# Renmusxd/IsingMonteCarlo

Measured on AMD Instinct MI355X. Metric: spin-op updates/sec (whole node), 32×32 TFIM, 1024 replicas at 1/2/4/8 GPUs, higher is better.
Workload: dtype u32 op words, f64 acceptance arithmetic

## Files before the change

isingmontecarlo_amd/csrc/sse_fast.hip.h:

```cpp
#pragma once

namespace sse {

#define SSE_FAST_MAX_VARS 4096u
#define LDS8(a) (reinterpret_cast<uint8_t *>(lds_raw)[(a)])
#define SSE_FAST_CLASS_J 0u
#define SSE_FAST_CLASS_G 1u
#define SSE_FAST_CLASS_H 2u

__device__ __forceinline__ uint32_t sel64(uint64_t mask, uint32_t a, uint32_t b) {
    uint32_t r;
    asm("v_cndmask_b32 %0, %1, %2, %3" : "=v"(r) : "v"(b), "v"(a), "s"(mask));
    return r;
}

__device__ __forceinline__ uint32_t bfi32(uint32_t mask, uint32_t a, uint32_t b) {
    uint32_t r;
    asm("v_bfi_b32 %0, %1, %2, %3" : "=v"(r) : "v"(mask), "v"(a), "v"(b));
    return r;
}

struct FastLds {
    uint32_t o_nb;
    uint32_t o_tab;
    uint32_t o_spin;
    uint32_t o_dummy;
    uint32_t end;
};
template <int W>
__host__ __device__ __forceinline__ FastLds fast_carve(const Lds<W> &L, const DevBatch &B) {
    FastLds F;
    uint32_t base = (L.o_edges + 3u) & ~3u;
    F.o_nb = base; base += 16;
    F.o_tab = base; base += B.Nb;
    F.o_spin = base; base += B.N;
    F.o_dummy = base; base += 64;
    F.end = base;
    return F;
}

__device__ __forceinline__ uint32_t fast_entry(const DevBatch &B, uint32_t b, uint32_t ce) {
    if (b < B.E) {
        const uint32_t a = ce & SSE_CE_VAR_MASK, c = (ce >> 15) & SSE_CE_VAR_MASK, pref = (ce >> 30) & 1u;
        return a | (c << 12) | ((pref ? 0x9u : 0x6u) << 24) | (3u << 28) | (SSE_FAST_CLASS_J << 30);
    }
    const uint32_t s1 = b - B.E;
    if (s1 < B.N) return s1 | (s1 << 12) | (0xFu << 24) | (1u << 28) | (SSE_FAST_CLASS_G << 30);
    const uint32_t v = s1 - B.N;
    return v | (v << 12) | ((B.hpos ? 0x8u : 0x1u) << 24) | (1u << 28) | (SSE_FAST_CLASS_H << 30);
}

template <int K>
__device__ __forceinline__ void diagonal_fast(const DevBatch &B, const Lds<4> &L, const FastLds &F, uint32_t r, const Rng &rng, double beta,
                                              uint32_t M, int &n_io, int &ntrans_io, uint32_t &gr, uint32_t fbmask) {
    constexpr int W = 4, NT = W * 64;
    constexpr uint32_t TS = (uint32_t)(NT * K);
    static_assert(K == 2 || K == 4, "rows p and p + 64 share one Philox call");
    const int tid = threadIdx.x, lane = tid & 63, wave = __builtin_amdgcn_readfirstlane(tid >> 6);
    uint32_t *ops = B.ops + (size_t)r * B.stride;
    const uint8_t *flipb = (fbmask ? B.flipb : reinterpret_cast<const uint8_t *>(B.ops)) + (size_t)r * B.stride;
    auto ld_word = [&](uint32_t idx) -> uint32_t {
        return row_ld(ops, idx) ^ ((uint32_t)*reinterpret_cast<const uint8_t *>(reinterpret_cast<const char *>(flipb) + (size_t)idx) & fbmask);
    };
    const uint32_t N = B.N, Nb = B.Nb, E = B.E;
    for (uint32_t i = tid; i < N; i += NT) LDSW(F.o_spin, i) = ((LDSW(L.o_state, i >> 5) >> (i & 31)) & 1u) * 0x01010101u;
    __syncthreads();

    const uint32_t ntiles = (M + TS - 1) / TS;
    int n_start = n_io, ntrans = 0;
    const uint32_t m_later = (uint32_t)((0x0101010100ull << (8 * wave)) & 0xFFFFFFFFull);
    const uint32_t m_earlier = 0x01010101u & ((1u << (8 * wave)) - 1u);
    const uint32_t spin_my = 4u * F.o_spin + (uint32_t)wave;
    const uint32_t markhi = (127u - (uint32_t)lane) << 1;

    const uint32_t dummy_w = F.o_dummy + (uint32_t)lane;
    auto evmask32 = [](uint32_t wd) -> uint32_t { return 0u - ((wd ^ (wd >> 2)) & 1u); };
    auto propagate = [&](const uint32_t (&wd)[K], uint32_t mask) {
        if (mask == 0u) return;
#pragma unroll
        for (int j = 0; j < K; ++j) {
            const uint32_t v = F.o_spin + (wd[j] >> 4) - 1u - E;
            atomicXor(&lds_raw[bfi32(evmask32(wd[j]), v, dummy_w)], mask);
        }
    };

    uint32_t wnext[K];
#pragma unroll
    for (int j = 0; j < K; ++j) wnext[j] = ld_word((uint32_t)(wave * 64 * K + j * 64 + lane));
    propagate(wnext, m_later);
    __syncthreads();
    const uint32_t lane2 = 2u * (uint32_t)lane;
    const uint32_t vM = vgpr_copy_u32(M), vM1 = vgpr_copy_u32(M + 1u), vzero = vgpr_copy_u32(0u);

    for (uint32_t tile = 0; tile < ntiles; ++tile) {
#if SSE_ROTATE_PRIO
        if ((tile & (SSE_ROTATE_PRIO - 1u)) == 0u) sse_set_prio((tile / SSE_ROTATE_PRIO) + blockIdx.x);
#endif
        uint32_t word[K];
#pragma unroll
        for (int j = 0; j < K; ++j) word[j] = wnext[j];
        const uint32_t pbase = tile * TS + (uint32_t)(wave * 64 * K + lane);
        {
            const uint32_t pn = (tile + 1 < ntiles ? pbase + TS : pbase);
#pragma unroll
            for (int j = 0; j < K; ++j) wnext[j] = ld_word(pn + (uint32_t)(j * 64));
        }
        const bool partial = tile * TS + TS > M;

        double un[K], nb[K];
        uint32_t cbv[K], neww[K], ent[K], bnd[K], rr1[K];
        uint64_t insm[K], remm[K], acc[K];
        {
            uint4 rnd = make_uint4(0, 0, 0, 0);
#pragma unroll
            for (int j = 0; j < K; ++j) {
                const uint32_t wd = word[j];
                if ((j & 1) == 0) rnd = rng.draw(SSE_TAG_DIAG, pbase + (uint32_t)(j * 64));
                const uint32_t r0 = (j & 1) ? rnd.z : rnd.x;
                rr1[j] = (j & 1) ? rnd.w : rnd.y;
                const uint64_t occm = sse_ballot(wd != 0u);
                bnd[j] = sel64(occm, (wd >> 4) - 1u, __umulhi(r0, Nb));
                ent[j] = LDSW(F.o_tab, bnd[j]);
            }
        }
        uint32_t sub0[K];
#pragma unroll
        for (int j = 0; j < K; ++j) {
            const uint32_t e = ent[j], inb = word[j] & 1u;
            const uint32_t va = e & 0xFFFu, vc = (e >> 12) & 0xFFFu;
            const uint32_t adr_a = spin_my + 4u * va, adr_c = spin_my + 4u * vc;
            const uint32_t mark = markhi | inb;
            const uint32_t ev32 = evmask32(word[j]);
            const uint32_t adr_w = bfi32(ev32, adr_a, 4u * dummy_w);
            LDS8(adr_w) = (uint8_t)mark;
            SSE_WAVE_FENCE();
            const uint32_t ea = LDS8(adr_a), ec = LDS8(adr_c);
            uint32_t sa, sc;
            const uint64_t dup = sse_ballot(((ea ^ mark) & ev32) != 0u);
            if (!dup) {
                sa = (ea ^ ((ea + lane2) >> 8)) & 1u;
                sc = (ec ^ ((ec + lane2) >> 8)) & 1u;
                SSE_WAVE_FENCE();
                LDS8(adr_w) = (uint8_t)(inb ^ 1u);
            } else {
                sa = ea & 1u; sc = ec & 1u;
                bool seen_a = false, seen_c = false;
                uint64_t m = sse_ballot(ev32 != 0u);
                while (m) {
                    const int Ls = __ffsll((long long)m) - 1;
                    m &= m - 1;
                    const bool later = lane > Ls;
                    const uint32_t vL = __builtin_amdgcn_readlane(va, Ls), inL = __builtin_amdgcn_readlane(inb, Ls);
                    if (va == vL) { sa = later ? (inL ^ 1u) : (seen_a ? sa : inL); seen_a = true; }
                    if (vc == vL) { sc = later ? (inL ^ 1u) : (seen_c ? sc : inL); seen_c = true; }
                    if (lane == Ls) LDS8(adr_a) = (uint8_t)(inL ^ 1u);
                }
                SSE_WAVE_FENCE();
            }
            sub0[j] = sa | (sc << 1);
        }
#pragma unroll
        for (int j = 0; j < K; ++j) {
            const uint32_t e = ent[j], wd = word[j];
            const uint32_t okbit = (e >> (24u + sub0[j])) & 1u;
            const uint32_t sub = sub0[j] & (e >> 28) & 3u;
            const double2 nbp = *reinterpret_cast<const double2 *>(&lds_raw[F.o_nb + 4u * (e >> 30)]);
            const double u = (double)rr1[j];
            insm[j] = sse_ballot(okbit > wd);
            if (partial) insm[j] &= sse_ballot(pbase + (uint32_t)(j * 64) < M);
            remm[j] = sse_ballot((wd & ~evmask32(wd)) != 0u);
            un[j] = u * nbp.y;
            nb[j] = nbp.x;
            cbv[j] = sel64(insm[j], vM, vM1);
            neww[j] = sel64(insm[j], ((bnd[j] + 1u) << 4) | sub | (sub << 2), vzero);
            acc[j] = 0ull;
        }

        int npref[K];
#pragma unroll
        for (int j = 0; j < K; ++j) npref[j] = n_start;
        int tot_all = 0, base = 0;
        bool first = true;
        for (;;) {
            int wtot = 0;
            bool changed = first;
#pragma unroll
            for (int j = 0; j < K; ++j) {
                const double t = (double)(int)(cbv[j] - (uint32_t)npref[j]);
                const uint64_t lt_ins = sse_ballot((double)rr1[j] * t < nb[j]);
                const uint64_t lt_rem = sse_ballot(un[j] < t);
                const uint64_t a = (lt_ins & insm[j]) | (lt_rem & remm[j]);
                changed |= a != acc[j];
                acc[j] = a;
                wtot += popc64(a & insm[j]) - popc64(a & remm[j]);
            }
            const int buf = gr & 1;
            if (lane == 0) { LDSI(L.o_tot, buf * W + wave) = wtot; LDSW(L.o_chg, buf * W + wave) = changed ? 1u : 0u; }
            __syncthreads();
            if (first) {
                propagate(word, m_earlier);
                if (tile + 1 < ntiles) propagate(wnext, m_later);
            }
            base = 0; tot_all = 0; uint32_t anychg = 0;
#pragma unroll
            for (int w2 = 0; w2 < W; ++w2) {
                const int t = __builtin_amdgcn_readfirstlane(LDSI(L.o_tot, buf * W + w2));
                if (w2 < wave) base += t;
                tot_all += t;
                anychg |= (uint32_t)__builtin_amdgcn_readfirstlane((int)LDSW(L.o_chg, buf * W + w2)) & 1u;
            }
            gr++;
            if (!first && !anychg) break;
            first = false;
            int run = n_start + base;
#pragma unroll
            for (int j = 0; j < K; ++j) {
                const uint64_t im = acc[j] & insm[j], rm = acc[j] & remm[j];
                const int ci = (int)__builtin_amdgcn_mbcnt_hi((uint32_t)(im >> 32), __builtin_amdgcn_mbcnt_lo((uint32_t)im, (uint32_t)run));
                const int cr = (int)__builtin_amdgcn_mbcnt_hi((uint32_t)(rm >> 32), __builtin_amdgcn_mbcnt_lo((uint32_t)rm, 0u));
                npref[j] = ci - cr;
                run += popc64(im) - popc64(rm);
            }
        }
        int dn = 0, dtr = 0;
#pragma unroll
        for (int j = 0; j < K; ++j) {
            const uint32_t fw = sel64(acc[j], neww[j], word[j]);
            row_st(ops, pbase + (uint32_t)(j * 64), fw);
            const uint64_t im = acc[j] & insm[j], rm = acc[j] & remm[j];
            const uint64_t trm = sse_ballot((ent[j] >> 30) == SSE_FAST_CLASS_G);
            dn += popc64(im) - popc64(rm);
            dtr += popc64(im & trm) - popc64(rm & trm);
        }
        ntrans += dtr;
        if (lane == 0 && (dtr | dn)) {
            const uint32_t ch = (tile * TS + (uint32_t)(wave * 64 * K)) / B.CH;
            if (dn) atomicAdd(&LDSW(L.o_chn, ch), (uint32_t)dn);
            if (dtr) atomicAdd(&LDSW(L.o_chtr, ch), (uint32_t)dtr);
        }
        n_start += tot_all;
    }
    __syncthreads();
    if (lane == 0) LDSI(L.o_tot, wave) = ntrans;
    __syncthreads();
    int dt = 0;
#pragma unroll
    for (int w2 = 0; w2 < W; ++w2) dt += LDSI(L.o_tot, w2);
    __syncthreads();
    ntrans_io += dt;
    n_io = n_start;
}

template <int K, int PHASE>
__global__ __launch_bounds__(256, 4) void sweep_fast_kernel(DevBatch B, SweepArgs A) {
    constexpr int W = 4, NT = W * 64;
    Lds<W> L;
    L.carve(B.N, B.nwords, B.lds_ufcap, B.E, B.has_long);
    const FastLds F = fast_carve<W>(L, B);
    const int tid = threadIdx.x;
    const uint32_t r = blockIdx.x;
#ifdef SSE_WG_TIMELINE
    if (tid == 0 && (B.dbg_flags & 32u)) { B.dbg[(size_t)r * 16 + 0] = __builtin_amdgcn_s_memrealtime(); B.dbg[(size_t)r * 16 + 2] = __builtin_amdgcn_s_getreg((4 << 0) | (0 << 6) | (31 << 11)); B.dbg[(size_t)r * 16 + 3] = __builtin_amdgcn_s_getreg((20 << 0) | (0 << 6) | (31 << 11)); }
#endif
    const double beta = A.beta ? A.beta[r] : 0.0;
    for (uint32_t i = tid; i < B.nwords; i += NT) LDSW(L.o_state, i) = B.state[(size_t)r * B.nwords + i];
    for (uint32_t i = tid; i < B.Nb; i += NT) LDSW(F.o_tab, i) = fast_entry(B, i, i < B.E ? B.edges_compact[i] : 0u);
    for (uint32_t i = tid; i < 2 * SSE_MAX_CHUNKS; i += NT) LDSW(L.o_chn, i) = B.chunks[(size_t)r * 2 * SSE_MAX_CHUNKS + i];
    if (tid < 4) {
        const double beta_nb = beta * (double)B.Nb;
        const double w = tid == 0 ? B.wJ : (tid == 1 ? B.gamma : (tid == 2 ? B.wh : 0.0));
        const double num = beta_nb * w;
        *reinterpret_cast<double *>(&lds_raw[F.o_nb + 4u * (uint32_t)tid]) = num * 4294967296.0;
        *reinterpret_cast<double *>(&lds_raw[F.o_nb + 4u * (uint32_t)tid + 2u]) = num * (1.0 / 4294967296.0);
    }
    __syncthreads();
    int n = (int)B.n[r], ntrans = (int)B.ntrans[r];
    uint32_t M = B.cutoff[r], err = B.err[r], gr = 0, last_out = 0;
    uint64_t epoch = B.epoch[r];
    uint64_t a4 = 0, a5 = 0;
    const uint32_t fbmask = (A.defer_flips && B.flipb && (A.domask & SSE_DO_DIAG) && !err && B.pend[r]) ? 0xFFu : 0u;
    for (uint64_t step = 0; step < A.nsteps; ++step) {
        if (err) break;
        if (A.domask & SSE_DO_DIAG) {
            const Rng rng = make_rng(B, r, epoch);
            diagonal_fast<K>(B, L, F, r, rng, beta, M, n, ntrans, gr, step == 0 ? fbmask : 0u);
            epoch++;
            a5 += M;
            if (A.domask & SSE_DO_GROW) {
                const uint32_t want = (uint32_t)n + (uint32_t)n / 2u;
                if (want > M) { if (want > B.cap) { err = 1u; break; } M = want; }
            }
        }
        if (A.domask & SSE_DO_LOOP) {
            __syncthreads();
            for (uint32_t i = tid; i < B.E; i += NT) LDSW(L.o_edges, i) = B.edges_compact[i];
            __syncthreads();
            const Rng rng = make_rng(B, r, epoch);
            last_out = loop_pass<W, true>(B, L, r, rng, M, n, gr, err);
            epoch++;
            a4 += last_out;
            if (err) break;
        }
    }
    __syncthreads();
    for (uint32_t i = tid; i < B.nwords; i += NT) B.state[(size_t)r * B.nwords + i] = LDSW(L.o_state, i);
    for (uint32_t i = tid; i < 2 * SSE_MAX_CHUNKS; i += NT) B.chunks[(size_t)r * 2 * SSE_MAX_CHUNKS + i] = LDSW(L.o_chn, i);
    if (tid == 0) {
        B.n[r] = (uint32_t)n; B.ntrans[r] = (uint32_t)ntrans; B.cutoff[r] = M; B.err[r] = err; B.epoch[r] = epoch;
        if (fbmask && A.nsteps) B.pend[r] = 0u;
        if (A.out_u32) A.out_u32[r] = last_out;
        uint64_t *acc = B.acc + (size_t)B.acc_row[r] * 8;
        acc[4] += a4; acc[5] += a5;
#ifdef SSE_WG_TIMELINE
        if (B.dbg_flags & 32u) B.dbg[(size_t)r * 16 + 1] = __builtin_amdgcn_s_memrealtime();
#endif
    }
}

}
```

isingmontecarlo_amd/csrc/sweep_fast.hip:

```cpp
#include "sse_device.hip.h"
namespace sse {
template <int K, int PHASE>
static hipError_t launch_fast_one(const LaunchCfg &c, const DevBatch &B, const SweepArgs &A) {
    hipError_t e = hipFuncSetAttribute(reinterpret_cast<const void *>(&sweep_fast_kernel<K, PHASE>), hipFuncAttributeMaxDynamicSharedMemorySize, (int)c.lds_bytes);
    if (e != hipSuccess) return e;
    hipLaunchKernelGGL((sweep_fast_kernel<K, PHASE>), dim3(B.R), dim3(256), c.lds_bytes, c.stream, B, A);
    return hipGetLastError();
}
hipError_t launch_sweep_fast(const LaunchCfg &c, const DevBatch &B, const SweepArgs &A) {
    if (c.W != 4 || c.mode != SSE_MODE_LDS_EDGES) return hipErrorInvalidValue;
    if (c.K == 4) return c.phase ? launch_fast_one<4, 1>(c, B, A) : launch_fast_one<4, 0>(c, B, A);
    if (c.K == 2) return launch_fast_one<2, 0>(c, B, A);
    return hipErrorInvalidValue;
}
}
```

Baseline: 162.5 billion.

## Replace f64 acceptance tests with exact integer thresholds in diagonal update

Adds an integer acceptance path. The insert test becomes a 64-bit multiply-add sign check against a precomputed constant, and the remove test compares an int against a threshold converted once per tile. This takes the f64 multiplies and compares out of the iterative prefix-sum fixed-point loop. It also packs the per-wave total and changed flag into one LDS word read as a single uint4, caches the decoded spin addresses, and tracks the chunk index incrementally instead of dividing every tile. The f64 path is kept for replicas whose capacity exceeds 2^21. The integer path must match the f64 decisions exactly, so rounding edge cases are a correctness risk.

```diff
diff --git a/isingmontecarlo_amd/csrc/sse_accept.h b/isingmontecarlo_amd/csrc/sse_accept.h
--- /dev/null
+++ b/isingmontecarlo_amd/csrc/sse_accept.h
@@ -0,0 +1,39 @@
+#pragma once
+#include <stdint.h>
+
+#if defined(__HIPCC__) || defined(__CUDACC__)
+#define SSE_ACCEPT_FN __host__ __device__ inline
+#else
+#define SSE_ACCEPT_FN inline
+#endif
+
+#define SSE_ACCEPT_MAX_DEN (1u << 21)
+#define SSE_ACCEPT_NEVER_INSERT 0x8000000000000000ull
+#define SSE_ACCEPT_NEVER_REMOVE 0x7FFFFFFF
+
+SSE_ACCEPT_FN uint64_t sse_accept_insert_const(double num) {
+    const double s = num * 4294967296.0;
+    if (!(s > 0.0)) return SSE_ACCEPT_NEVER_INSERT;
+    if (s >= 9223372036854775808.0) return 1ull;
+    uint64_t nbi = (uint64_t)s;
+    if ((double)nbi < s) nbi += 1ull;
+    return SSE_ACCEPT_NEVER_INSERT - nbi;
+}
+
+SSE_ACCEPT_FN bool sse_accept_insert(uint32_t rr1, uint32_t den, uint64_t c) {
+    return (int32_t)(((uint64_t)rr1 * (uint64_t)den + c) >> 32) >= 0;
+}
+
+SSE_ACCEPT_FN int32_t sse_accept_remove_threshold(uint32_t rr1, double num_lo) {
+    const double un = (double)rr1 * num_lo;
+#if defined(__HIP_DEVICE_COMPILE__)
+    int32_t r;
+    asm("v_cvt_i32_f64 %0, %1" : "=v"(r) : "v"(un));
+    return r;
+#else
+    if (!(un < 2147483647.0)) return SSE_ACCEPT_NEVER_REMOVE;
+    return un > 0.0 ? (int32_t)un : 0;
+#endif
+}
+
+SSE_ACCEPT_FN bool sse_accept_remove(int32_t den, int32_t thr) { return den > thr; }
diff --git a/isingmontecarlo_amd/csrc/sse_fast.hip.h b/isingmontecarlo_amd/csrc/sse_fast.hip.h
--- a/isingmontecarlo_amd/csrc/sse_fast.hip.h
+++ b/isingmontecarlo_amd/csrc/sse_fast.hip.h
@@ -1,4 +1,5 @@
 #pragma once
+#include "sse_accept.h"
 
 namespace sse {
 
@@ -22,6 +23,7 @@
 
 struct FastLds {
     uint32_t o_nb;
+    uint32_t o_xch;
     uint32_t o_tab;
     uint32_t o_spin;
     uint32_t o_dummy;
@@ -30,8 +32,10 @@
 template <int W>
 __host__ __device__ __forceinline__ FastLds fast_carve(const Lds<W> &L, const DevBatch &B) {
     FastLds F;
+    static_assert(4 * W >= 3 + 8, "o_xch: eight words behind an alignment gap of up to three, inside o_tot + o_chg");
     uint32_t base = (L.o_edges + 3u) & ~3u;
     F.o_nb = base; base += 16;
+    F.o_xch = (L.o_tot + 3u) & ~3u;
     F.o_tab = base; base += B.Nb;
     F.o_spin = base; base += B.N;
     F.o_dummy = base; base += 64;
@@ -50,7 +54,7 @@
     return v | (v << 12) | ((B.hpos ? 0x8u : 0x1u) << 24) | (1u << 28) | (SSE_FAST_CLASS_H << 30);
 }
 
-template <int K>
+template <int K, bool F64>
 __device__ __forceinline__ void diagonal_fast(const DevBatch &B, const Lds<4> &L, const FastLds &F, uint32_t r, const Rng &rng, double beta,
                                               uint32_t M, int &n_io, int &ntrans_io, uint32_t &gr, uint32_t fbmask) {
     constexpr int W = 4, NT = W * 64;
@@ -73,32 +77,33 @@
     const uint32_t spin_my = 4u * F.o_spin + (uint32_t)wave;
     const uint32_t markhi = (127u - (uint32_t)lane) << 1;
 
-    const uint32_t dummy_w = F.o_dummy + (uint32_t)lane;
+    const uint32_t dummy_b = 4u * (F.o_dummy + (uint32_t)lane);
     auto evmask32 = [](uint32_t wd) -> uint32_t { return 0u - ((wd ^ (wd >> 2)) & 1u); };
-    auto propagate = [&](const uint32_t (&wd)[K], uint32_t mask) {
+    const uint32_t spin_b = 4u * (F.o_spin - 1u - E);
+    auto decode = [&](uint32_t wd) -> uint32_t { return bfi32(evmask32(wd), spin_b + 4u * (wd >> 4), dummy_b); };
+    auto propagate = [&](const uint32_t (&vb)[K], uint32_t mask) {
         if (mask == 0u) return;
 #pragma unroll
-        for (int j = 0; j < K; ++j) {
-            const uint32_t v = F.o_spin + (wd[j] >> 4) - 1u - E;
-            atomicXor(&lds_raw[bfi32(evmask32(wd[j]), v, dummy_w)], mask);
-        }
+        for (int j = 0; j < K; ++j) atomicXor(reinterpret_cast<uint32_t *>(reinterpret_cast<char *>(lds_raw) + vb[j]), mask);
     };
 
-    uint32_t wnext[K];
-#pragma unroll
-    for (int j = 0; j < K; ++j) wnext[j] = ld_word((uint32_t)(wave * 64 * K + j * 64 + lane));
-    propagate(wnext, m_later);
+    uint32_t wnext[K], vnext[K];
+#pragma unroll
+    for (int j = 0; j < K; ++j) { wnext[j] = ld_word((uint32_t)(wave * 64 * K + j * 64 + lane)); vnext[j] = decode(wnext[j]); }
+    propagate(vnext, m_later);
     __syncthreads();
     const uint32_t lane2 = 2u * (uint32_t)lane;
     const uint32_t vM = vgpr_copy_u32(M), vM1 = vgpr_copy_u32(M + 1u), vzero = vgpr_copy_u32(0u);
+    const uint32_t vnever_hi = vgpr_copy_u32((uint32_t)(SSE_ACCEPT_NEVER_INSERT >> 32)), vnever_thr = vgpr_copy_u32((uint32_t)SSE_ACCEPT_NEVER_REMOVE);
+    uint32_t ch = (uint32_t)(wave * 64 * K) / B.CH, chpos = (uint32_t)(wave * 64 * K) % B.CH;
 
     for (uint32_t tile = 0; tile < ntiles; ++tile) {
 #if SSE_ROTATE_PRIO
         if ((tile & (SSE_ROTATE_PRIO - 1u)) == 0u) sse_set_prio((tile / SSE_ROTATE_PRIO) + blockIdx.x);
 #endif
-        uint32_t word[K];
-#pragma unroll
-        for (int j = 0; j < K; ++j) word[j] = wnext[j];
+        uint32_t word[K], vcur[K];
+#pragma unroll
+        for (int j = 0; j < K; ++j) { word[j] = wnext[j]; vcur[j] = vnext[j]; }
         const uint32_t pbase = tile * TS + (uint32_t)(wave * 64 * K + lane);
         {
             const uint32_t pn = (tile + 1 < ntiles ? pbase + TS : pbase);
@@ -107,9 +112,13 @@
         }
         const bool partial = tile * TS + TS > M;
 
+        uint32_t cbv[K], neww[K], ent[K], bnd[K], rr1[K];
+        uint64_t acci[K], accr[K];
+        uint32_t chi[K];
+        uint32_t clo[K];
+        int32_t thr[K];
         double un[K], nb[K];
-        uint32_t cbv[K], neww[K], ent[K], bnd[K], rr1[K];
-        uint64_t insm[K], remm[K], acc[K];
+        uint64_t insm[K], remm[K];
         {
             uint4 rnd = make_uint4(0, 0, 0, 0);
 #pragma unroll
@@ -130,13 +139,13 @@
             const uint32_t va = e & 0xFFFu, vc = (e >> 12) & 0xFFFu;
             const uint32_t adr_a = spin_my + 4u * va, adr_c = spin_my + 4u * vc;
             const uint32_t mark = markhi | inb;
-            const uint32_t ev32 = evmask32(word[j]);
-            const uint32_t adr_w = bfi32(ev32, adr_a, 4u * dummy_w);
+            const uint32_t adr_w = vcur[j] + (uint32_t)wave;
+            const uint64_t evm = sse_ballot(vcur[j] != dummy_b);
             LDS8(adr_w) = (uint8_t)mark;
             SSE_WAVE_FENCE();
             const uint32_t ea = LDS8(adr_a), ec = LDS8(adr_c);
             uint32_t sa, sc;
-            const uint64_t dup = sse_ballot(((ea ^ mark) & ev32) != 0u);
+            const uint64_t dup = sse_ballot(ea != mark) & evm;
             if (!dup) {
                 sa = (ea ^ ((ea + lane2) >> 8)) & 1u;
                 sc = (ec ^ ((ec + lane2) >> 8)) & 1u;
@@ -145,7 +154,7 @@
             } else {
                 sa = ea & 1u; sc = ec & 1u;
                 bool seen_a = false, seen_c = false;
-                uint64_t m = sse_ballot(ev32 != 0u);
+                uint64_t m = evm;
                 while (m) {
                     const int Ls = __ffsll((long long)m) - 1;
                     m &= m - 1;
@@ -164,81 +173,100 @@
             const uint32_t e = ent[j], wd = word[j];
             const uint32_t okbit = (e >> (24u + sub0[j])) & 1u;
             const uint32_t sub = sub0[j] & (e >> 28) & 3u;
-            const double2 nbp = *reinterpret_cast<const double2 *>(&lds_raw[F.o_nb + 4u * (e >> 30)]);
-            const double u = (double)rr1[j];
-            insm[j] = sse_ballot(okbit > wd);
-            if (partial) insm[j] &= sse_ballot(pbase + (uint32_t)(j * 64) < M);
-            remm[j] = sse_ballot((wd & ~evmask32(wd)) != 0u);
-            un[j] = u * nbp.y;
-            nb[j] = nbp.x;
-            cbv[j] = sel64(insm[j], vM, vM1);
-            neww[j] = sel64(insm[j], ((bnd[j] + 1u) << 4) | sub | (sub << 2), vzero);
-            acc[j] = 0ull;
+            const uint4 cls = *reinterpret_cast<const uint4 *>(&lds_raw[F.o_nb + 4u * (e >> 30)]);
+            const double num_lo = __hiloint2double((int)cls.w, (int)cls.z);
+            uint64_t im = sse_ballot(okbit > wd);
+            if (partial) im &= sse_ballot(pbase + (uint32_t)(j * 64) < M);
+            const uint64_t rm = sse_ballot(wd != 0u) & ~sse_ballot(vcur[j] != dummy_b);
+            if constexpr (F64) {
+                un[j] = (double)rr1[j] * num_lo;
+                nb[j] = __hiloint2double((int)cls.y, (int)cls.x);
+                insm[j] = im; remm[j] = rm;
+            } else {
+                clo[j] = cls.x;
+                chi[j] = sel64(im, cls.y, vnever_hi);
+                thr[j] = (int32_t)sel64(rm, (uint32_t)sse_accept_remove_threshold(rr1[j], num_lo), vnever_thr);
+            }
+            cbv[j] = sel64(im, vM, vM1);
+            neww[j] = sel64(im, ((bnd[j] + 1u) << 4) | sub | (sub << 2), vzero);
+            acci[j] = 0ull; accr[j] = 0ull;
         }
 
         int npref[K];
 #pragma unroll
         for (int j = 0; j < K; ++j) npref[j] = n_start;
-        int tot_all = 0, base = 0;
+        int tot_all = 0, base = 0, wtot = 0;
         bool first = true;
         for (;;) {
-            int wtot = 0;
-            bool changed = first;
+            wtot = 0;
+            uint64_t diff = 0ull;
 #pragma unroll
             for (int j = 0; j < K; ++j) {
-                const double t = (double)(int)(cbv[j] - (uint32_t)npref[j]);
-                const uint64_t lt_ins = sse_ballot((double)rr1[j] * t < nb[j]);
-                const uint64_t lt_rem = sse_ballot(un[j] < t);
-                const uint64_t a = (lt_ins & insm[j]) | (lt_rem & remm[j]);
-                changed |= a != acc[j];
-                acc[j] = a;
-                wtot += popc64(a & insm[j]) - popc64(a & remm[j]);
-            }
-            const int buf = gr & 1;
-            if (lane == 0) { LDSI(L.o_tot, buf * W + wave) = wtot; LDSW(L.o_chg, buf * W + wave) = changed ? 1u : 0u; }
+                const int t = (int)(cbv[j] - (uint32_t)npref[j]);
+                uint64_t ai, ar;
+                if constexpr (F64) {
+                    const double td = (double)t;
+                    ai = sse_ballot((double)rr1[j] * td < nb[j]) & insm[j];
+                    ar = sse_ballot(un[j] < td) & remm[j];
+                } else {
+                    ai = sse_ballot(sse_accept_insert(rr1[j], (uint32_t)t, ((uint64_t)chi[j] << 32) | clo[j]));
+                    ar = sse_ballot(sse_accept_remove(t, thr[j]));
+                }
+                diff |= (ai ^ acci[j]) | (ar ^ accr[j]);
+                acci[j] = ai; accr[j] = ar;
+                wtot += popc64(ai) - popc64(ar);
+            }
+            const bool changed = first | (diff != 0ull);
+            const uint32_t xch = F.o_xch + 4u * (gr & 1u);
+            if (lane == 0) LDSW(xch, wave) = ((uint32_t)wtot << 1) | (changed ? 1u : 0u);
             __syncthreads();
             if (first) {
-                propagate(word, m_earlier);
-                if (tile + 1 < ntiles) propagate(wnext, m_later);
-            }
-            base = 0; tot_all = 0; uint32_t anychg = 0;
+                propagate(vcur, m_earlier);
+#pragma unroll
+                for (int j = 0; j < K; ++j) vnext[j] = decode(wnext[j]);
+                if (tile + 1 < ntiles) propagate(vnext, m_later);
+            }
+            const uint4 xw = *reinterpret_cast<const uint4 *>(&lds_raw[xch]);
+            const int x4[W] = {__builtin_amdgcn_readfirstlane((int)xw.x), __builtin_amdgcn_readfirstlane((int)xw.y),
+                               __builtin_amdgcn_readfirstlane((int)xw.z), __builtin_amdgcn_readfirstlane((int)xw.w)};
+            base = 0; tot_all = 0;
 #pragma unroll
             for (int w2 = 0; w2 < W; ++w2) {
-                const int t = __builtin_amdgcn_readfirstlane(LDSI(L.o_tot, buf * W + w2));
+                const int t = x4[w2] >> 1;
                 if (w2 < wave) base += t;
                 tot_all += t;
-                anychg |= (uint32_t)__builtin_amdgcn_readfirstlane((int)LDSW(L.o_chg, buf * W + w2)) & 1u;
-            }
+            }
+            const uint32_t anychg = (uint32_t)(x4[0] | x4[1] | x4[2] | x4[3]) & 1u;
             gr++;
             if (!first && !anychg) break;
             first = false;
             int run = n_start + base;
 #pragma unroll
             for (int j = 0; j < K; ++j) {
-                const uint64_t im = acc[j] & insm[j], rm = acc[j] & remm[j];
+                const uint64_t im = acci[j], rm = accr[j];
                 const int ci = (int)__builtin_amdgcn_mbcnt_hi((uint32_t)(im >> 32), __builtin_amdgcn_mbcnt_lo((uint32_t)im, (uint32_t)run));
                 const int cr = (int)__builtin_amdgcn_mbcnt_hi((uint32_t)(rm >> 32), __builtin_amdgcn_mbcnt_lo((uint32_t)rm, 0u));
                 npref[j] = ci - cr;
                 run += popc64(im) - popc64(rm);
             }
         }
-        int dn = 0, dtr = 0;
+        const int dn = wtot;
+        int dtr = 0;
 #pragma unroll
         for (int j = 0; j < K; ++j) {
-            const uint32_t fw = sel64(acc[j], neww[j], word[j]);
+            const uint32_t fw = sel64(acci[j] | accr[j], neww[j], word[j]);
             row_st(ops, pbase + (uint32_t)(j * 64), fw);
-            const uint64_t im = acc[j] & insm[j], rm = acc[j] & remm[j];
             const uint64_t trm = sse_ballot((ent[j] >> 30) == SSE_FAST_CLASS_G);
-            dn += popc64(im) - popc64(rm);
-            dtr += popc64(im & trm) - popc64(rm & trm);
+            dtr += popc64(acci[j] & trm) - popc64(accr[j] & trm);
         }
         ntrans += dtr;
         if (lane == 0 && (dtr | dn)) {
-            const uint32_t ch = (tile * TS + (uint32_t)(wave * 64 * K)) / B.CH;
             if (dn) atomicAdd(&LDSW(L.o_chn, ch), (uint32_t)dn);
             if (dtr) atomicAdd(&LDSW(L.o_chtr, ch), (uint32_t)dtr);
         }
         n_start += tot_all;
+        chpos += TS;
+        while (chpos >= B.CH) { chpos -= B.CH; ch++; }
     }
     __syncthreads();
     if (lane == 0) LDSI(L.o_tot, wave) = ntrans;
@@ -251,7 +279,7 @@
     n_io = n_start;
 }
 
-template <int K, int PHASE>
+template <int K, int PHASE, bool F64>
 __global__ __launch_bounds__(256, 4) void sweep_fast_kernel(DevBatch B, SweepArgs A) {
     constexpr int W = 4, NT = W * 64;
     Lds<W> L;
@@ -270,7 +298,8 @@
         const double beta_nb = beta * (double)B.Nb;
         const double w = tid == 0 ? B.wJ : (tid == 1 ? B.gamma : (tid == 2 ? B.wh : 0.0));
         const double num = beta_nb * w;
-        *reinterpret_cast<double *>(&lds_raw[F.o_nb + 4u * (uint32_t)tid]) = num * 4294967296.0;
+        if constexpr (F64) *reinterpret_cast<double *>(&lds_raw[F.o_nb + 4u * (uint32_t)tid]) = num * 4294967296.0;
+        else *reinterpret_cast<uint64_t *>(&lds_raw[F.o_nb + 4u * (uint32_t)tid]) = sse_accept_insert_const(num);
         *reinterpret_cast<double *>(&lds_raw[F.o_nb + 4u * (uint32_t)tid + 2u]) = num * (1.0 / 4294967296.0);
     }
     __syncthreads();
@@ -283,7 +312,7 @@
         if (err) break;
         if (A.domask & SSE_DO_DIAG) {
             const Rng rng = make_rng(B, r, epoch);
-            diagonal_fast<K>(B, L, F, r, rng, beta, M, n, ntrans, gr, step == 0 ? fbmask : 0u);
+            diagonal_fast<K, F64>(B, L, F, r, rng, beta, M, n, ntrans, gr, step == 0 ? fbmask : 0u);
             epoch++;
             a5 += M;
             if (A.domask & SSE_DO_GROW) {
diff --git a/isingmontecarlo_amd/csrc/sweep_fast.hip b/isingmontecarlo_amd/csrc/sweep_fast.hip
--- a/isingmontecarlo_amd/csrc/sweep_fast.hip
+++ b/isingmontecarlo_amd/csrc/sweep_fast.hip
@@ -1,16 +1,20 @@
 #include "sse_device.hip.h"
 namespace sse {
-template <int K, int PHASE>
+template <int K, int PHASE, bool F64>
 static hipError_t launch_fast_one(const LaunchCfg &c, const DevBatch &B, const SweepArgs &A) {
-    hipError_t e = hipFuncSetAttribute(reinterpret_cast<const void *>(&sweep_fast_kernel<K, PHASE>), hipFuncAttributeMaxDynamicSharedMemorySize, (int)c.lds_bytes);
+    hipError_t e = hipFuncSetAttribute(reinterpret_cast<const void *>(&sweep_fast_kernel<K, PHASE, F64>), hipFuncAttributeMaxDynamicSharedMemorySize, (int)c.lds_bytes);
     if (e != hipSuccess) return e;
-    hipLaunchKernelGGL((sweep_fast_kernel<K, PHASE>), dim3(B.R), dim3(256), c.lds_bytes, c.stream, B, A);
+    hipLaunchKernelGGL((sweep_fast_kernel<K, PHASE, F64>), dim3(B.R), dim3(256), c.lds_bytes, c.stream, B, A);
     return hipGetLastError();
 }
 hipError_t launch_sweep_fast(const LaunchCfg &c, const DevBatch &B, const SweepArgs &A) {
     if (c.W != 4 || c.mode != SSE_MODE_LDS_EDGES) return hipErrorInvalidValue;
-    if (c.K == 4) return c.phase ? launch_fast_one<4, 1>(c, B, A) : launch_fast_one<4, 0>(c, B, A);
-    if (c.K == 2) return launch_fast_one<2, 0>(c, B, A);
+    const bool f64 = B.cap > SSE_ACCEPT_MAX_DEN;
+    if (c.K == 4) {
+        if (f64) return c.phase ? launch_fast_one<4, 1, true>(c, B, A) : launch_fast_one<4, 0, true>(c, B, A);
+        return c.phase ? launch_fast_one<4, 1, false>(c, B, A) : launch_fast_one<4, 0, false>(c, B, A);
+    }
+    if (c.K == 2) return f64 ? launch_fast_one<2, 0, true>(c, B, A) : launch_fast_one<2, 0, false>(c, B, A);
     return hipErrorInvalidValue;
 }
 }
```

Measured after the change: 169.6 billion, median of 6. +4.3%, better.
